# CIawevy/FreeFine

Measured on AMD Instinct MI355X. Metric: edited images/sec/GPU @512px 50-step DDIM, higher is better.
Workload: dtype bf16x3

## Files before the change

### __graft_entry__.py

```python
import os
import subprocess
import sys

ROOT = os.path.dirname(os.path.abspath(__file__))
if ROOT not in sys.path:
    sys.path.insert(0, ROOT)

HIPCC = os.environ.get("HIPCC", "/opt/rocm/bin/hipcc")
LIB = os.path.join(ROOT, "freefine_amd", "libfreefine_hip.so")
CSRC = os.path.join(ROOT, "freefine_amd", "csrc")
OBJDIR = os.path.join(ROOT, "build", "obj")
UNITS = [("capi_igemm.hip", []), ("capi_attn.hip", []), ("capi.hip", []), ("capi_splat.hip", []),
         ("attn_x3w.hip", ["-mllvm", "-amdgpu-mfma-vgpr-form", "-fno-slp-vectorize"]), ("attn_causal.hip", []), ("dift.hip", []), ("imgprep.hip", []),
         ("inception.hip", [])]
COMMON = ["--offload-arch=gfx950", "-O3", "-std=c++17", "-fPIC"]


def _stale(target, deps):
    if not os.path.exists(target):
        return True
    t = os.path.getmtime(target)
    return any(os.path.getmtime(d) > t for d in deps)


def build(force=False):
    deps = [os.path.join(CSRC, f) for f in os.listdir(CSRC)] + [os.path.join(ROOT, "include", "freefine_hip.h")]
    if force or _stale(LIB, deps):
        os.makedirs(OBJDIR, exist_ok=True)
        procs = []
        for src, extra in UNITS:
            obj = os.path.join(OBJDIR, src.replace(".hip", ".o"))
            cmd = [HIPCC] + COMMON + extra + ["-c", "-o", obj, os.path.join(CSRC, src)]
            print("[build]", " ".join(cmd), flush=True)
            procs.append((cmd, obj, subprocess.Popen(cmd, cwd=ROOT)))
        for cmd, obj, pr in procs:
            if pr.wait() != 0:
                raise subprocess.CalledProcessError(pr.returncode, cmd)
        cmd = [HIPCC, "--offload-arch=gfx950", "-shared", "-fPIC", "-o", LIB] + [obj for _, obj, _ in procs]
        print("[build]", " ".join(cmd), flush=True)
        subprocess.check_call(cmd, cwd=ROOT)
    import freefine_amd
    from freefine_amd import _lib
    _lib.load()
    import oracle.attention_modulation, oracle.masks, oracle.pipeline, oracle.scheduler, oracle.sd_unet, oracle.sd_vae
    print(f"[build] {LIB} exports {len(_lib.SYMBOLS)} symbols; oracle importable", flush=True)


def smoke():
    import numpy as np
    import torch
    assert torch.cuda.is_available(), "smoke() needs a GPU"
    from freefine_amd import _lib
    _lib.load()
    sys.path.insert(0, os.path.join(ROOT, "tests"))
    from golden_cases import edit_cases, mask_inputs, oracle_pipe, synth_images
    from test_pipeline_gpu import make_pipe
    dev = torch.device("cuda:0")
    ori_img, coarse, _ = synth_images()
    ori, tgt, *_ = mask_inputs()
    name, unet_name, kw = edit_cases()[0]
    kw = dict(kw)
    text, gs, eta = kw.pop("guidance_text"), kw.pop("guidance_scale"), kw.pop("eta")
    model = make_pipe(dev, unet_name, "edit", graph=True)
    img = model.FreeFine_generation(ori_img, ori, coarse, tgt, text, gs, eta, verbose=True, seed=42, return_intermediates=True, **kw)
    with torch.no_grad():
        o_img, _, o_traj = oracle_pipe(unet_name).freefine_generation(ori_img, ori, coarse, tgt, text, gs, eta, seed=42, **kw)
    dev_max = max((a.float().cpu() - b).abs().max().item() for a, b in zip(model.last_intermediates, o_traj))
# ... 10 lines not shown
```

### freefine_amd/_lib.py

```python
import ctypes as C
import os

_HERE = os.path.dirname(os.path.abspath(__file__))
LIB_PATH = os.environ.get("FREEFINE_HIP_LIB") or os.path.join(_HERE, "libfreefine_hip.so")

FFN_F32, FFN_BF16, FFN_BF16X3, FFN_FP8 = 0, 1, 2, 3
IG_OUT_SILU, IG_OUT_F32, IG_GEGLU, IG_OUT_TRANSPOSED, IG_OUT_PAIR, IG_OUT_GELU, IG_OUT_RELU, IG_OUT_KV64 = 1, 2, 4, 8, 16, 32, 64, 128
IG_OUT_QGELU = 256
ELT_RELU, ELT_ADD, ELT_GELU = 0, 1, 2
ATT_MAXP, ATT_MAXB = 4, 16
ATT_HEAD_RULE, ATT_UNIFORM_SEL1, ATT_UNIFORM_SEL0, ATT_CAUSAL = 1, 2, 4, 8
NORM_SILU, NORM_OUT_PAIR = 1, 2
IMGPREP_MAX_SIDE = 4096
IMGPREP_MAX_TAPS = 2 * 3 * IMGPREP_MAX_SIDE + 1
BOX_NMS_MAX = 16384
KEEP_NONE, KEEP_SUM_LT128, KEEP_GT128 = 0, 1, 2
CHAIN_MAXL, CHAIN_MAXW = 8, 1024
CONV_RELU = 1
POOL_MAX, POOL_AVG_VALID = 0, 1


class IgemmDesc(C.Structure):
    _fields_ = [
        ("A", C.c_void_p), ("W", C.c_void_p), ("out", C.c_void_p),
# ... 67 lines not shown
    ]


class CoarseEditDesc(C.Structure):
    _fields_ = [
        ("src_img", C.c_void_p), ("src_mask", C.c_void_p), ("bg", C.c_void_p), ("hole_img", C.c_void_p), ("hole_mask", C.c_void_p), ("inv", C.c_void_p),
        ("final_img", C.c_void_p), ("tmask", C.c_void_p), ("trans_hole", C.c_void_p),
        ("B", C.c_int), ("H", C.c_int), ("W", C.c_int), ("mask_c", C.c_int), ("hole_mask_c", C.c_int),
    ]


class Conv2dDesc(C.Structure):
    _fields_ = [
        ("x", C.c_void_p), ("w", C.c_void_p), ("bias", C.c_void_p), ("out", C.c_void_p),
        ("B", C.c_int), ("Hin", C.c_int), ("Win", C.c_int), ("Cin", C.c_int), ("N", C.c_int),
        ("KH", C.c_int), ("KW", C.c_int), ("stride", C.c_int), ("pad_h", C.c_int), ("pad_w", C.c_int),
        ("ldx", C.c_int), ("ldo", C.c_int), ("Kpad", C.c_int), ("flags", C.c_int),
    ]


_vp, _i, _f, _l = C.c_void_p, C.c_int, C.c_float, C.c_long
SYMBOLS = {
    "ffn_version": (_i, []),
    "ffn_last_error": (C.c_char_p, []),
    "ffn_device_info": (_i, [_i, C.c_char_p, _i]),
    "ffn_graph_launch": (_i, [_vp, _vp]),
    "ffn_igemm": (_i, [_vp, _i, C.POINTER(IgemmDesc)]),
    "ffn_conv3x3_n4": (_i, [_vp, _i, _vp, _vp, _vp, _vp, _i, _i, _i, _i]),
    "ffn_split_pair": (_i, [_vp, _vp, _vp, _l, _i, _i]),
    "ffn_groupnorm_f8": (_i, [_vp, _vp, _vp, _vp, _vp, _i, _i, _i, _i, _i, _f, _i, _f, _vp, _vp, _vp]),
    "ffn_attn": (_i, [_vp, _i, C.POINTER(AttnDesc)]),
    "ffn_attn_kernel_name": (_i, [_i, C.POINTER(AttnDesc), C.c_char_p, _i]),
    "ffn_igemm_tune": (_i, [_vp, _i, C.POINTER(IgemmDesc)]),
    "ffn_igemm_tune_entry_ints": (_i, []),
    "ffn_igemm_tune_export": (_i, [C.POINTER(C.c_int), _i]),
    "ffn_igemm_tune_import": (_i, [C.POINTER(C.c_int), _i]),
    "ffn_igemm_tune_stamp": (_i, []),
    "ffn_igemm_tune_clear": (_i, []),
    "ffn_igemm_tune_enable": (_i, [_i]),
    "ffn_igemm_num_configs": (_i, []),
    "ffn_igemm_force_config": (_i, [_i]),
    "ffn_igemm_kernel_name": (_i, [_i, C.POINTER(IgemmDesc), C.c_char_p, _i]),
    "ffn_attn_presplit": (_i, [_vp, _vp, _vp, _vp, _vp, _i, _i, _i, _i, _i]),
    "ffn_attn_variant": (_i, [_i, _i, C.POINTER(C.c_int), C.POINTER(C.c_int)]),
    "ffn_gn_nchunk": (_i, [_i]),
    "ffn_gn_fused": (_i, [_i, _i, _i, _i]),
    "ffn_gn_stats": (_i, [_vp, _i, _vp, _vp, _vp, _i, _i, _i, _i, _f, _vp, _vp, _vp]),
    "ffn_gn_apply": (_i, [_vp, _i, _vp, _vp, _vp, _vp, _i, _i, _i, _i]),
    "ffn_groupnorm": (_i, [_vp, _i, _vp, _vp, _vp, _vp, _i, _i, _i, _i, _f, _i, _vp, _vp, _vp]),
    "ffn_groupnorm_pair_raw": (_i, [_vp, _vp, _vp, _vp, _vp, _vp, _i, _i, _i, _i, _f, _i, _vp, _vp, _vp]),
    "ffn_layernorm": (_i, [_vp, _i, _vp, _vp, _vp, _vp, _i, _i, _f]),
    "ffn_layernorm_pair": (_i, [_vp, _vp, _vp, _vp, _vp, _i, _i, _f]),
    "ffn_softmax_rows": (_i, [_vp, _i, _vp, _vp, _l, _i, _f]),
    "ffn_pool_layernorm": (_i, [_vp, _i, _vp, _vp, _vp, _vp, _vp, _i, _i, _i, _f, _i]),
    "ffn_cosine_rows": (_i, [_vp, _vp, _vp, _vp, _i, _i, _i]),
    "ffn_cfg_masked": (_i, [_vp, _vp, _vp, _vp, _f, _vp, _l, _i]),
    "ffn_ddim_inv_step": (_i, [_vp, _vp, _vp, _f, _f, _f, _f, _vp, _vp, _l]),
    "ffn_ddim_ctrl_step": (_i, [_vp, C.POINTER(CtrlStepDesc)]),
    "ffn_pack_nchw": (_i, [_vp, _i, C.POINTER(PackDesc)]),
    "ffn_nhwc_to_nchw_f32": (_i, [_vp, _vp, _vp, _i, _i, _i, _i]),
    "ffn_concat": (_i, [_vp, _i, _vp, _vp, _vp, _l, _i, _i]),
    "ffn_timestep_embed": (_i, [_vp, _i, _vp, _vp, _vp, _i, _i, _i]),
    "ffn_transpose": (_i, [_vp, _i, _vp, _vp, _i, _i, _i, _i, _i]),
    "ffn_cast": (_i, [_vp, _i, _i, _vp, _vp, _l]),
    "ffn_eltwise": (_i, [_vp, _i, _i, _vp, _vp, _vp, _l]),
    "ffn_resize_bilinear": (_i, [_vp, _i, _vp, _vp, _i, _i, _i, _i, _i, _i, _i]),
    "ffn_splat_lift": (_i, [_vp, _vp, _vp, _vp, _i, _i, _i, _f, _f]),
    "ffn_splat_project": (_i, [_vp, _vp, _vp, _i, C.POINTER(SplatXform)]),
    "ffn_splat_bin": (_i, [_vp, _i, _vp, _i, _f, _i, _i, _vp, _vp, _vp]),
    "ffn_splat_render": (_i, [_vp, _vp, _vp, _vp, _vp, _f, _i, _i, _i, _vp, _vp, _vp]),
    "ffn_splat_ids": (_i, [_vp, _vp, _vp, _vp, _f, _i, _i, _i, _vp]),
    "ffn_splat_correspond": (_i, [_vp, _vp, _vp, _i, _i, _i, _vp, _i, _vp, _vp]),
    "ffn_geo_project": (_i, [_vp, _vp, C.POINTER(C.c_float), _f, _i, _i, _vp, _vp]),
    "ffn_splat_composite": (_i, [_vp, _vp, _vp, _vp, _vp, _f, _f, _i, _i, _i, _i, _i, _vp]),
    "ffn_mesh_cover": (_i, [_vp, _vp, _vp, _i, _i, _vp]),
    "ffn_embed_tokens": (_i, [_vp, _i, _vp, _vp, _vp, _vp, _l, _i, _i, _i]),
    "ffn_embed_tokens_ln": (_i, [_vp, _i, _vp, _vp, _vp, _vp, _vp, _vp, _l, _i, _i, _i, _f]),
    "ffn_affine_chain": (_i, [_vp, _vp, _vp, _vp, _i, _i, C.POINTER(C.c_int), _i, _f, _f]),
    "ffn_dift_match": (_i, [_vp, C.POINTER(DiftDesc)]),
    "ffn_dift_workspace_bytes": (_l, [_i, _i, _i, _i]),
    "ffn_sift_base": (_i, [_vp, _vp, _vp, _i, _i, _i]),
    "ffn_gauss_blur_f32": (_i, [_vp, _vp, _vp, _vp, _i, _i, _vp, _i]),
    "ffn_decimate2_f32": (_i, [_vp, _vp, _vp, _i, _i]),
    "ffn_sift_extrema": (_i, [_vp, _vp, _vp, _i, _i, _vp, _i, _vp, C.POINTER(C.c_int)]),
    "ffn_sift_refine_orient": (_i, [_vp, _vp, _vp, _i, _i, _i, _vp, _i, _vp]),
    "ffn_sift_describe": (_i, [_vp, _vp, _i, _i, _i, _vp, _i, _vp, _vp]),
    "ffn_knn2_u8": (_i, [_vp, _vp, _i, _vp, _i, _vp, _vp]),
    "ffn_resize_pil_bilinear_u8": (_i, [_vp, _vp, _vp, _vp, _i, _i, _i, _i, _i, _vp, _vp, _i, _vp, _vp, _i]),
    "ffn_resize_pil_u8": (_i, [_vp, C.POINTER(ResizePilDesc)]),
    "ffn_resize_taps8_u8": (_i, [_vp, _vp, _vp, _i, _i, _i, _i, _i, _i, _vp, _vp, _vp, _vp]),
    "ffn_resize_gather_u8": (_i, [_vp, _vp, _vp, _i, _i, _i, _i, _i, _i, _vp, _vp, _i]),
    "ffn_dilate_u8": (_i, [_vp, _vp, _vp, _vp, _i, _i, _i, _i, _i]),
    "ffn_mask_bbox_u8": (_i, [_vp, _vp, _vp, _i, _i, _i, _i]),
    "ffn_coarse_edit_2d": (_i, [_vp, C.POINTER(CoarseEditDesc)]),
    "ffn_vit_patch_rows": (_i, [_vp, _i, _vp, _vp, _vp, _i, _i, _i, _i, _i]),
    "ffn_vit_patch_rows_pair": (_i, [_vp, _vp, _vp, _vp, _i, _i, _i, _i, _i]),
    "ffn_sam_patch_rows": (_i, [_vp, _i, _vp, _vp, _i, _i, _i, _i, _i, _i, C.POINTER(C.c_float), C.POINTER(C.c_float)]),
    "ffn_sam_patch_rows_pair": (_i, [_vp, _vp, _vp, _i, _i, _i, _i, _i, _i, C.POINTER(C.c_float), C.POINTER(C.c_float)]),
    "ffn_hyper_masks": (_i, [_vp, _vp, _vp, _vp, _i, _i, _i, _i]),
    "ffn_upsample_bicubic": (_i, [_vp, _vp, _vp, _vp, _i, _i, _i, _i, _i]),
    "ffn_upsample_bicubic_stats": (_i, [_vp, _vp, _vp, _vp, _i, _i, _i, _i, _i, _f]),
    "ffn_box_nms": (_i, [_vp, _vp, _vp, _i, _f]),
    "ffn_image_to_nhwc": (_i, [_vp, _i, _vp, _vp, _l, _i]),
    "ffn_nhwc_to_image": (_i, [_vp, _i, _vp, _vp, _i, _i, _i]),
    "ffn_conv2d": (_i, [_vp, _i, C.POINTER(Conv2dDesc)]),
    "ffn_pool2d": (_i, [_vp, _i, _vp, _vp, _i, _i, _i, _i, _i, _i, _i, _i, _i]),
# ... 33 lines not shown
```

### freefine_amd/csrc/capi.hip

```cpp
#include <stdlib.h>
#include <string.h>

#include "capi_common.h"
#include "conv_small.h"
#include "elementwise.h"
#include "norms.h"

__thread char g_err[512] = "";

extern "C" int ffn_version(void) { return 16; }
extern "C" const char* ffn_last_error(void) { return g_err; }
extern "C" int ffn_device_info(int device, char* name, int name_len) {
    hipDeviceProp_t prop;
    hipError_t e = hipGetDeviceProperties(&prop, device);
    if (e != hipSuccess) return fail(FFN_EHIP, "hipGetDeviceProperties: %s", hipGetErrorString(e));
    if (name && name_len > 0) {
        strncpy(name, prop.gcnArchName, name_len - 1);
        name[name_len - 1] = 0;
    }
    return prop.multiProcessorCount;
}

extern "C" int ffn_graph_launch(void* stream, void* graph_exec) {
    REQUIRE(graph_exec, "graph_launch: null graph");
    hipError_t e = hipGraphLaunch(reinterpret_cast<hipGraphExec_t>(graph_exec), reinterpret_cast<hipStream_t>(stream));
    if (e != hipSuccess) return fail(FFN_EHIP, "hipGraphLaunch: %s", hipGetErrorString(e));
    return FFN_OK;
}

extern "C" int ffn_split_pair(void* stream, const float* src, void* dst, long rows, int C, int ld_src) {
    REQUIRE(src && dst && rows > 0 && C > 0 && C % 4 == 0 && ld_src >= C && ld_src % 4 == 0, "split_pair: bad arguments (C=%d, ld_src=%d)", C, ld_src);
    REQUIRE(aligned16(src) && aligned16(dst), "split_pair: pointers must be 16-byte aligned");
    if (C % 8 == 0) LAUNCH(split_pair8_kernel, dim3(grid_for(rows * (C / 8))), dim3(256), 0, reinterpret_cast<hipStream_t>(stream), src, (bf16*)dst, rows, C, ld_src);
    else LAUNCH(split_pair_kernel, dim3(grid_for(rows * (C / 4))), dim3(256), 0, reinterpret_cast<hipStream_t>(stream), src, (bf16*)dst, rows, C, ld_src);
    return check_launch("split_pair");
}
extern "C" int ffn_conv3x3_n4(void* stream, int dtype, const void* x, const float* w, const float* bias, float* out, int B, int H, int W, int Cin) {
    REQUIRE(dtype == FFN_F32 || dtype == FFN_BF16, "conv3x3_n4: fp32 or bf16 activations");
    REQUIRE(x && w && out && aligned16(x) && aligned16(w) && aligned16(out) && (!bias || aligned16(bias)), "conv3x3_n4: null / unaligned pointer");
    REQUIRE(B > 0 && H > 0 && W > 0 && Cin > 0 && Cin % 16 == 0 && Cin <= 448, "conv3x3_n4: B=%d H=%d W=%d Cin=%d (Cin %% 16 == 0, <= 448)", B, H, W, Cin);
    hipStream_t s = reinterpret_cast<hipStream_t>(stream);
    const long npix = (long)B * H * W;
    const int lds = 36 * Cin * 4;
    dim3 grid((unsigned)((npix + 63) / 64));
    int rc;
    if (dtype == FFN_F32) {
        if ((rc = set_lds(conv3x3_n4_kernel<float>, lds))) return rc;
        LAUNCH(conv3x3_n4_kernel<float>, grid, dim3(256), lds, s, (const float*)x, w, bias, out, B, H, W, Cin);
    } else {
        if ((rc = set_lds(conv3x3_n4_kernel<bf16>, lds))) return rc;
        LAUNCH(conv3x3_n4_kernel<bf16>, grid, dim3(256), lds, s, (const bf16*)x, w, bias, out, B, H, W, Cin);
    }
    return check_launch("conv3x3_n4");
}

extern "C" int ffn_eltwise(void* stream, int dtype, int op, const void* a, const void* b, void* y, long n) {
    REQUIRE(dtype == FFN_F32 || dtype == FFN_BF16, "eltwise: bad dtype %d", dtype);
    REQUIRE(op == FFN_ELT_RELU || op == FFN_ELT_ADD || op == FFN_ELT_GELU, "eltwise: bad op %d", op);
    REQUIRE(a && y && (op != FFN_ELT_ADD || b), "eltwise: null operand");
    REQUIRE(n > 0 && n % 4 == 0, "eltwise: n=%ld must be a positive multiple of 4", n);
    hipStream_t s = reinterpret_cast<hipStream_t>(stream);
    const long n4 = n / 4;
    const int grid = grid_for(n4);
// ... 274 lines not shown
```

### freefine_amd/ops.py

```python
import ctypes as CT
import math

import os
import threading

import torch

from . import _lib as L


def _dt(t):
    if t.dtype == torch.float32:
        return L.FFN_F32
    if t.dtype == torch.bfloat16:
        return L.FFN_BF16
    raise TypeError(f"unsupported dtype {t.dtype}")


def epc(dtype):
    return 4 if dtype == torch.float32 else 8


def kstage(dtype):
    return 8 * epc(dtype)
# ... 302 lines not shown
    d.a_lo = (32 if d.x3 == 2 else K) if x3 else 0
    odt = torch.float32 if x3 else x.dtype
    d.rows_per_batch = rows_per_batch or M
    d.ldrb = rowbias.stride(0) if rowbias is not None else 0
    flags = 0
    n_out = N
    if silu:
        flags |= L.IG_OUT_SILU
    if gelu:
        flags |= L.IG_OUT_GELU
    if relu:
        flags |= L.IG_OUT_RELU
    if qgelu:
        flags |= L.IG_OUT_QGELU
    if geglu:
        flags |= L.IG_GEGLU
        n_out = N // 2
    if out_f32:
        flags |= L.IG_OUT_F32
    if transposed_ld is not None:
        flags |= L.IG_OUT_TRANSPOSED
        nb = M // d.rows_per_batch
        if out is None:
            alloc = torch.zeros if transposed_ld > d.rows_per_batch else torch.empty
            out = alloc(nb, N, transposed_ld, dtype=odt, device=x.device)
        d.ldo = transposed_ld
    elif out_pair:
        assert x3 and out is None
        flags |= L.IG_OUT_PAIR
        out = _mark_pair(torch.empty(*x.shape[:-1], 2 * n_out, dtype=torch.bfloat16, device=x.device), n_out)
        d.ldo = 2 * n_out
    else:
        if out is None:
            out = torch.empty(*x.shape[:-1], n_out, dtype=torch.float32 if out_f32 else odt, device=x.device)
        d.ldo = out.stride(-2) if out.ndim > 1 else n_out
    assert xa.stride(-1) == 1 and out.stride(-1) == 1 and (residual is None or residual.stride(-1) == 1), "linear: x, out and residual need contiguous columns"
    d.ldr = (residual.stride(-2) if residual.ndim > 1 else residual.shape[-1]) if residual is not None else 0
    d.out = out.data_ptr()
    if kv64_from is not None:
        assert x3 and residual is None and rowbias is None and not (silu or gelu or relu or qgelu or geglu or out_pair)
        flags |= L.IG_OUT_KV64
        d.kv64_from = int(kv64_from)
        splitk = 1
    d.flags, d.alpha, d.conv = flags, alpha, 0
    if splitk == 0 and _invariant():
        splitk = 1
    d.splitk, d.ws, d.ws_bytes = splitk, _workspace(x.device).data_ptr(), WS_BYTES
    if _PROF is None:
        L.check(lib.ffn_igemm(_stream(), dcode, CT.byref(d)), "ffn_igemm")
    else:
        esz = x.element_size()
        L.check(_timed(_igemm_name(lib, dcode, d), 2.0 * M * N * K, esz * (M * K + N * K + M * n_out),
                       lambda: lib.ffn_igemm(_stream(), dcode, CT.byref(d))), "ffn_igemm")
    return out


def conv3x3(x, w, bias, B, Hin, Win, Cin, *, stride=1, pad=1, upsample=False, out=None, residual=None, rowbias=None,
            rowbias_ld=None, out_f32=False, Hout=None, Wout=None, splitk=0, relu=False):
    lib = L.load()
    He, We = (Hin * 2, Win * 2) if upsample else (Hin, Win)
    if Hout is None:
        Hout = (He + 2 * pad - 3) // stride + 1
        Wout = (We + 2 * pad - 3) // stride + 1
    N = w.shape[0]
    d = L.IgemmDesc()
    x3 = is_x3(w)
    f8 = is_f8(w)
    if f8:
        assert x.dtype == torch.uint8 and x.shape[-1] == w._ffn_f8[0] and out_f32 is False
        Cin = x.shape[-1]
        xa = x
    elif x3 and pair_width(x) is not None:
        assert pair_width(x) == Cin
        xa = x
    else:
        xa = split_pair(x, Cin) if x3 else x
    dcode = L.FFN_FP8 if f8 else (L.FFN_BF16X3 if x3 else _dt(x))
    odt = torch.float32 if x3 else (torch.bfloat16 if f8 else x.dtype)
    d.A, d.W = xa.data_ptr(), w.data_ptr()
    d.bias, d.rowbias, d.residual = _p(bias), _p(rowbias), _p(residual)
    d.M, d.N, d.K, d.Kpad = B * Hout * Wout, N, 9 * Cin, w.shape[1]
    d.lda = 2 * Cin if x3 else Cin
    d.x3 = int(w._ffn_x3) if x3 else 0
    d.a_lo = (32 if d.x3 == 2 else Cin) if x3 else 0
    d.rows_per_batch = Hout * Wout
    d.ldrb = (rowbias_ld or rowbias.stride(0)) if rowbias is not None else 0
    if out is None:
        out = torch.empty(B, Hout * Wout, N, dtype=torch.float32 if out_f32 else odt, device=x.device)
    assert xa.is_contiguous(), "conv3x3: x must be contiguous (a column view of a wider buffer has no pixel stride the kernels could follow)"
    assert out.stride(-1) == 1 and (residual is None or residual.stride(-1) == 1), "conv3x3: out and residual need contiguous columns"
    d.out, d.ldo = out.data_ptr(), out.stride(-2)
    d.ldr = residual.stride(-2) if residual is not None else 0
    d.Hin, d.Win, d.Cin, d.Hout, d.Wout = Hin, Win, Cin, Hout, Wout
    d.stride, d.pad, d.upsample = stride, pad, 1 if upsample else 0
    d.flags, d.alpha, d.conv = (L.IG_OUT_F32 if out_f32 else 0) | (L.IG_OUT_RELU if relu else 0), (w._ffn_f8[1] if f8 else 1.0), 1
    if splitk == 0 and _invariant():
        splitk = 1
    d.splitk, d.ws, d.ws_bytes = splitk, _workspace(x.device).data_ptr(), WS_BYTES
    if _PROF is None:
        L.check(lib.ffn_igemm(_stream(), dcode, CT.byref(d)), "ffn_igemm(conv)")
    else:
        esz = x.element_size()
        k_real = 9 * getattr(x, "_ffn_f8_act", Cin)
        L.check(_timed(_igemm_name(lib, dcode, d), 2.0 * d.M * N * k_real, esz * (x.numel() + N * d.K + d.M * N),
                       lambda: lib.ffn_igemm(_stream(), dcode, CT.byref(d))), "ffn_igemm(conv)")
    return out
# ... 1143 lines not shown
```

### freefine_amd/unet.py

```python
import ctypes as CT
import weakref

import torch

from . import _lib as L
from . import ops
from .config import UNetConfig


class _Res:
    pass


class HipUNet:
    def __init__(self, cfg: UNetConfig, state, dtype=torch.bfloat16, device="cuda:0", x3=False, fp8_conv=False):
        assert not x3 or dtype == torch.float32, "split-bf16 mode keeps fp32 activations"
        assert not fp8_conv or dtype == torch.bfloat16, "fp8 convolutions are an option of the bf16 fast mode"
        self.x3 = bool(x3)
        self.fp8_conv = bool(fp8_conv)
        self.cfg, self.dtype, self.device = cfg, dtype, torch.device(device)
        self.in_channels = cfg.in_channels
        self.hook, self.controller = "edit", None
        self._graphs = {}
        self._capture_stream = None
# ... 534 lines not shown
            vt2 = torch.cat([vt[..., :Sk], vt[rr][..., :Sk]], dim=2).contiguous()
            return ops.attention(q, k2, vt2, t.heads, scale, plan["passes"], Sk=2 * Sk, C=t.C, x3=self.x3, out_pair=self.x3)
        return ops.attention(q, k, vt, t.heads, scale, plan["passes"], Sk=Sk, C=t.C, w_dev=self.cg_dev if plan["needs_cg"] else None, x3=self.x3,
                             out_pair=self.x3, kv_images=kv_images)

    def _kv_buffers(self, B, S, C, ldv):
        ru = self._reuse
        i = ru["cursor"]
        ru["cursor"] = i + 1
        if ru.get("static_ready"):
            return ru["static_bufs"][i]
        k_ref, vt_ref = ru["state"][2 * i], ru["state"][2 * i + 1]
        nr = k_ref.shape[0]
        assert tuple(k_ref.shape) == (nr, S, C) and tuple(vt_ref.shape) == (nr, C, ldv), (tuple(k_ref.shape), tuple(vt_ref.shape), (S, C, ldv))
        qk = torch.empty(B + nr, S, 2 * C, dtype=self.dtype, device=self.device)
        vt = torch.empty(B + nr, C, ldv, dtype=self.dtype, device=self.device)
        qk[B:, :, C:].copy_(k_ref)
        vt[B:].copy_(vt_ref)
        if ru.get("static") is not None:
            ru["static_bufs"].append((qk, vt))
            ru["static"] += [qk[B:, :, C:], vt[B:]]
        return qk, vt

    def _transformer_block(self, t, x, B, H, W, place, kv_text, out=None, drop=None, tb=0):
        S, C = H * W, t.C
        res0 = x
        ru = self._reuse
        h = self._gn(x, t.norm, 1e-6, False)
        h = ops.linear(h, t.proj_in[0], t.proj_in[1], K=C)
        y = ops.layernorm(h, *t.ln[0], pair=self.x3)
        ldv = (S + 7) // 8 * 8
        if ru is not None and ru["mode"] == "replay_kv" and tb >= ru["kv_from"]:
            qk, vt = self._kv_buffers(B, S, C, ldv)
            ops.linear(y, t.w_qk1, None, K=C, out=qk[:B])
            ops.linear(y, t.w_v1, None, K=C, rows_per_batch=S, transposed_ld=ldv, out=vt[:B])
            self._kv_ext = True
            a = self._attention(t, False, place, qk[:B], qk[..., C:], vt, 2 * C, B, S, S, plan=self._self_plan(t, place, B, S))
            self._kv_ext = False
        else:
            plan = self._self_plan(t, place, B, S, drop_ref_queries=drop is not None)
            rec = ru is not None and ru["mode"] == "record" and ru.get("kv_from") is not None and tb >= ru["kv_from"]
            img = self.x3 and not rec and (plan is None or plan["kind"] != "shared_kv") and \
                ops.kv_images_ok(C // t.heads, S, S, None if plan is None else plan["passes"], B * max(S * 2 * C, C * ldv) * 4)
            qk = ops.linear(y, t.w_qk1, None, K=C, kv64_from=C if img else None)
            vt = ops.linear(y, t.w_v1, None, K=C, rows_per_batch=S, transposed_ld=ldv, kv64_from=0 if img else None)
            if rec:
                self.last_kv.append((qk[..., C:], vt))
            a = self._attention(t, False, place, qk, qk[..., C:], vt, 2 * C, B, S, S, plan=plan, kv_images=img)
        if drop is not None:
            idx, kv_text = drop
            h, res0, B = h.index_select(0, idx), res0.index_select(0, idx), idx.shape[0]
            self._in_phase_a = True
        h = ops.linear(a, t.o1[0], t.o1[1], K=C, residual=h)
        y = ops.layernorm(h, *t.ln[1], pair=self.x3)
        q = ops.linear(y, t.w_q2, None, K=C)
        k2, vt2 = kv_text
        a = self._attention(t, True, place, q, k2, vt2, C, B, S, k2.shape[1])
        h = ops.linear(a, t.o2[0], t.o2[1], K=C, residual=h)
        y = ops.layernorm(h, *t.ln[2], pair=self.x3)
        y = ops.linear(y, t.ff1[0], t.ff1[1], K=C, geglu=True, out_pair=self.x3)
        h = ops.linear(y, t.ff2[0], t.ff2[1], K=4 * C, residual=h, out_pair=self.x3 and C % 32 == 0)
        return ops.linear(h, t.proj_out[0], t.proj_out[1], K=C, residual=res0, out=out)

    def _run(self, sample, text_kv, stop_up=None):
        cfg = self.cfg
        B, _, H, W = sample.shape
        dt = self.dtype
        ru = self._reuse
        replay = ru is not None and ru["mode"] == "replay"
        record = ru is not None and ru["mode"] == "record"
        replay_kv = ru is not None and ru["mode"] == "replay_kv"
        BB = B
        if replay:
            sample = sample.index_select(0, ru["idx_a"])
            B = sample.shape[0]
            text_kv = list(ru["text_kv_a"][:self.join_block_tb(ru["join"])]) + list(text_kv[self.join_block_tb(ru["join"]):])
        if replay_kv:
            sample = sample.index_select(0, ru["idx_a"])
            B = sample.shape[0]
            text_kv = ru["text_kv_a"]
            ru["cursor"] = 0
        if record and ru.get("kv_from") is not None:
            self.last_kv = []
        self._in_phase_a = replay
        ti = iter(text_kv)
        tb = 0
        te = ops.timestep_embed(self.t_dev, self.freq, BB, dt, flip=cfg.flip_sin_to_cos)
        e1 = ops.linear(te, self.te1[0], self.te1[1], K=self.te1[2], silu=True)
        e2 = ops.linear(e1, self.te2[0], self.te2[1], K=self.te2[2], silu=True)
        temb_all = ops.linear(e2, self.temb_w, self.temb_b, K=self.te2[0].shape[0], out_f32=True)
        temb_full = temb_all
        temb_all = temb_all[:B]
        x = ops.pack_nchw(sample, list(range(B)), self.cin_pad, dt)
        x = ops.conv3x3(x, self.conv_in[0], self.conv_in[1], B, H, W, self.cin_pad)
        skips = [(x, H, W)]
        n = len(self.down)
        for i, blk in enumerate(self.down):
            for j, r in enumerate(blk.res):
                x = self._resblock(r, x, B, H, W, temb_all)
                if blk.attn:
                    x = self._transformer_block(blk.attn[j], x, B, H, W, "down", next(ti), tb=tb)
                    tb += 1
                skips.append((x, H, W))
            if blk.down is not None:
                C = x.shape[-1]
                x = ops.conv3x3(x, blk.down[0], blk.down[1], B, H, W, C, stride=2)
                H, W = (H + 1) // 2, (W + 1) // 2
                skips.append((x, H, W))
# ... 54 lines not shown
```

### include/freefine_hip.h

```cpp
#ifndef FREEFINE_HIP_H
#define FREEFINE_HIP_H
#include <stdint.h>
#ifdef __cplusplus
extern "C" {
#endif

enum { FFN_F32 = 0, FFN_BF16 = 1, FFN_BF16X3 = 2 ,
       FFN_FP8 = 3  };
enum { FFN_OK = 0, FFN_EINVAL = -22, FFN_ENOSYS = -38, FFN_EHIP = -5, FFN_ENOSPC = -28 };

int ffn_version(void);
const char* ffn_last_error(void);
int ffn_device_info(int device, char* name, int name_len);
int ffn_graph_launch(void* stream, void* graph_exec);

enum {
    FFN_IG_OUT_SILU = 1 << 0,
    FFN_IG_OUT_F32 = 1 << 1,
    FFN_IG_GEGLU = 1 << 2,
    FFN_IG_OUT_TRANSPOSED = 1 << 3,
    FFN_IG_OUT_PAIR = 1 << 4,
    FFN_IG_OUT_GELU = 1 << 5,
    FFN_IG_OUT_KV64 = 1 << 7,
    FFN_IG_OUT_RELU = 1 << 6,
// ... 55 lines not shown
    const void* k;
    const void* vt;
    void* out;
    const float* w_dev;
    int Bo, S, Sk, heads, D;
    int ldq, ldk, ldvt, ldo;
    float scale;
    int npass;
    int out_pair;
    int kv_pair;
    ffn_attn_entry e[FFN_ATT_MAXP * FFN_ATT_MAXB];
} ffn_attn_desc;
int ffn_attn(void* stream, int dtype, const ffn_attn_desc* d);
int ffn_attn_presplit(void* stream, const float* k, const float* vt, void* k_pair, void* vt_pair, int rows, int Sk, int heads, int ldk, int ldvt);
int ffn_attn_variant(int dtype, int D, int* dp, int* qf);
int ffn_attn_kernel_name(int dtype, const ffn_attn_desc* d, char* buf, int len);

enum { FFN_ELT_RELU = 0, FFN_ELT_ADD = 1, FFN_ELT_GELU = 2 };
int ffn_eltwise(void* stream, int dtype, int op, const void* a, const void* b, void* y, long n);
int ffn_resize_bilinear(void* stream, int dtype, const void* x, void* y, int B, int Hin, int Win, int Hout, int Wout, int C, int relu);

typedef struct ffn_splat_xform {
    float center[3], translate[3], rotate[9] , scale[3];
    float tan_half_fov;
} ffn_splat_xform;
int ffn_splat_lift(void* stream, const float* depth, const int* idx, float* pts, int n, int W, int H, float fx, float fy);
int ffn_splat_project(void* stream, const float* pts, float* proj, int n, const ffn_splat_xform* x);
int ffn_splat_bin(void* stream, int fill, const float* proj, int n, float radius, int W, int H, int* counts, const int* offs, int* list);
int ffn_splat_render(void* stream, const float* proj, const float* rgb, const int* offs, const int* list, float radius, int K, int W, int H,
                     float* image, int* idx_sum, uint8_t* covered);
int ffn_splat_ids(void* stream, const float* proj, const int* offs, const int* list, float radius, int K, int W, int H, int* ids);
int ffn_splat_correspond(void* stream, const float* proj, const int* idx, int n, int W, int H, const int* ids, int K, float* map, uint8_t* visible);

int ffn_geo_project(void* stream, const float* depth, const float* pose, float focal, int H, int W, float* tcoords, float* proj);
int ffn_splat_composite(void* stream, const float* proj, const float* feat, const int* offs, const int* list, float radius, float tau, int K,
                        int C, int H, int W, int round_half, float* out);
int ffn_mesh_cover(void* stream, const float* tcoords, const uint8_t* mask, int H, int W, uint8_t* cover);

enum { FFN_NORM_SILU = 1, FFN_NORM_OUT_PAIR = 2 };
int ffn_gn_nchunk(int HW);
int ffn_gn_fused(int B, int HW, int C, int G);
int ffn_gn_stats(void* stream, int dtype, const void* x, const float* gamma, const float* beta, int B, int HW, int C, int G,
                 float eps, float* partial_ws, float* scale, float* shift);
int ffn_gn_apply(void* stream, int dtype, const void* x, void* y, const float* scale, const float* shift, int B, int HW,
                 int C, int silu);
int ffn_groupnorm(void* stream, int dtype, const void* x, void* y, const float* gamma, const float* beta, int B, int HW, int C, int G,
                  float eps, int silu, float* partial_ws, float* scale, float* shift);
int ffn_groupnorm_pair_raw(void* stream, const void* x, void* y_pair, void* yraw_pair, const float* gamma, const float* beta, int B, int HW, int C, int G,
                           float eps, int silu, float* partial_ws, float* scale, float* shift);
int ffn_layernorm(void* stream, int dtype, const void* x, void* y, const float* gamma, const float* beta, int M, int C,
                  float eps);
int ffn_layernorm_pair(void* stream, const float* x, void* y, const float* gamma, const float* beta, int M, int C, float eps);
int ffn_softmax_rows(void* stream, int dtype, const void* x, void* y, long M, int N, float scale);
int ffn_pool_layernorm(void* stream, int dtype, const void* x, const int* ids, void* y, const float* gamma, const float* beta, int N, int S, int C, float eps,
                       int pair);
int ffn_cosine_rows(void* stream, const float* a, const float* b, float* out, int B, int P, int b_rows);

int ffn_cfg_masked(void* stream, const float* eps_u, const float* eps_c, const float* mask, float cfg, float* eps, long n,
                   int HW);
int ffn_ddim_inv_step(void* stream, const float* eps, const float* x, float c_bt, float c_at, float c_an, float c_bn,
                      float* x_next, float* pred_x0, long n);
typedef struct ffn_ctrl_step_desc {
    const float* eps;
    const float* x;
    const float* noise;
    const float* m;
    const float* om;
    float* x_prev;
    float* pred_x0;
    float c_bt, c_at, c_ap, c_dir;
    float c_dirm[8], stdv[8];
    int row_masked[8];
    int rows, CHW, HW;
} ffn_ctrl_step_desc;
int ffn_ddim_ctrl_step(void* stream, const ffn_ctrl_step_desc* d);

typedef struct ffn_pack_desc {
    const float* src;
    void* dst;
    int src_row[16];
    int B, Cl, CP, HW;
} ffn_pack_desc;
int ffn_pack_nchw(void* stream, int dtype, const ffn_pack_desc* d);
int ffn_nhwc_to_nchw_f32(void* stream, const float* src, float* dst, int B, int HW, int C, int ld);
int ffn_concat(void* stream, int dtype, const void* a, const void* b, void* out, long rows, int C1, int C2);
int ffn_timestep_embed(void* stream, int dtype, const float* t_dev, const float* freq, void* out, int B, int half, int flip);
int ffn_transpose(void* stream, int dtype, const void* src, void* dst, int B, int R, int C, int ld_src, int ld_dst);
int ffn_cast(void* stream, int src_dtype, int dst_dtype, const void* src, void* dst, long n);
int ffn_embed_tokens(void* stream, int dtype, const int* ids, const float* table, const float* pos, void* out, long M, int S, int C, int V);
int ffn_embed_tokens_ln(void* stream, int dtype, const int* ids, const float* table, const float* pos, void* out, const float* gamma, const float* beta, long M,
                        int S, int C, int V, float eps);
#define FFN_CHAIN_MAXL 8
#define FFN_CHAIN_MAXW 1024
int ffn_affine_chain(void* stream, const float* x, const float* params, float* out, int B, int ldx, const int* dims, int L, float shift, float scale);
int ffn_image_to_nhwc(void* stream, int dtype, const uint8_t* img, void* dst, long npix, int CP);
int ffn_nhwc_to_image(void* stream, int dtype, const void* src, float* dst, int B, int HW, int ld);

typedef struct ffn_dift_desc {
    const void* src;
    const void* tgt;
    const int* kps;
    void* ws;
    int* out_rc;
    float* out_cos;
    long ws_bytes;
    long es;
// ... 88 lines not shown
```

Before: 1.976.

## Fuse LayerNorm into the cross-attention Q projection GEMM for C=320

Adds a dedicated kernel that computes LayerNorm on fp32 rows, splits the result into bf16 hi/lo pairs held in registers (AGPR/VGPR), and runs a bf16x3 MFMA GEMM against the Q weight. The weight is streamed through a three-slot LDS ring using buffer-to-LDS loads. The UNet transformer block uses it for the cross-attention query when the hidden width is 320. This removes the separate layernorm kernel and the round trip of the normalized pair tensor through memory. In exchange it adds a hand-scheduled kernel with a K restricted to 320, tight register pressure and explicit waitcnt tuning.

```diff
diff --git a/__graft_entry__.py b/__graft_entry__.py
--- a/__graft_entry__.py
+++ b/__graft_entry__.py
@@ -12,7 +12,7 @@
 OBJDIR = os.path.join(ROOT, "build", "obj")
 UNITS = [("capi_igemm.hip", []), ("capi_attn.hip", []), ("capi.hip", []), ("capi_splat.hip", []),
          ("attn_x3w.hip", ["-mllvm", "-amdgpu-mfma-vgpr-form", "-fno-slp-vectorize"]), ("attn_causal.hip", []), ("dift.hip", []), ("imgprep.hip", []),
-         ("inception.hip", [])]
+         ("inception.hip", []), ("igemm_as.hip", ["-mllvm", "-amdgpu-mfma-vgpr-form", "-fno-slp-vectorize"])]
 COMMON = ["--offload-arch=gfx950", "-O3", "-std=c++17", "-fPIC"]
 
 
diff --git a/freefine_amd/_lib.py b/freefine_amd/_lib.py
--- a/freefine_amd/_lib.py
+++ b/freefine_amd/_lib.py
@@ -143,6 +143,7 @@
     "ffn_layernorm": (_i, [_vp, _i, _vp, _vp, _vp, _vp, _i, _i, _f]),
     "ffn_layernorm_pair": (_i, [_vp, _vp, _vp, _vp, _vp, _i, _i, _f]),
     "ffn_softmax_rows": (_i, [_vp, _i, _vp, _vp, _l, _i, _f]),
+    "ffn_ln_igemm": (_i, [_vp, _vp, _i, _vp, _vp, _f, _i, _i, _vp, _i, _vp, _i, _vp, _i]),
     "ffn_pool_layernorm": (_i, [_vp, _i, _vp, _vp, _vp, _vp, _vp, _i, _i, _i, _f, _i]),
     "ffn_cosine_rows": (_i, [_vp, _vp, _vp, _vp, _i, _i, _i]),
     "ffn_cfg_masked": (_i, [_vp, _vp, _vp, _vp, _f, _vp, _l, _i]),
diff --git a/freefine_amd/csrc/capi.hip b/freefine_amd/csrc/capi.hip
--- a/freefine_amd/csrc/capi.hip
+++ b/freefine_amd/csrc/capi.hip
@@ -8,7 +8,7 @@
 
 __thread char g_err[512] = "";
 
-extern "C" int ffn_version(void) { return 16; }
+extern "C" int ffn_version(void) { return 17; }
 extern "C" const char* ffn_last_error(void) { return g_err; }
 extern "C" int ffn_device_info(int device, char* name, int name_len) {
     hipDeviceProp_t prop;
diff --git a/freefine_amd/csrc/igemm_as.h b/freefine_amd/csrc/igemm_as.h
--- /dev/null
+++ b/freefine_amd/csrc/igemm_as.h
@@ -0,0 +1,237 @@
+#pragma once
+#include "common.h"
+
+typedef __attribute__((ext_vector_type(16))) float f32x16;
+typedef __attribute__((address_space(3))) void* as_lptr_t;
+
+struct LnIgemmParams {
+    const float* x;
+    const float* gamma;
+    const float* beta;
+    const void* W;
+    const float* bias;
+    void* out;
+    int M, N, ldx, Kpad, ldo;
+    int wbytes, obytes;
+    float eps;
+};
+
+#define LNIG_SB_FREE (0x002 | 0x004 | 0x010 | 0x020 | 0x040 | 0x400)
+constexpr int LNIG_SLOT = 10 * 4096;
+constexpr int LNIG_RING = 3;
+constexpr int LNIG_OFF_B = LNIG_RING * LNIG_SLOT;
+constexpr int LNIG_STG_ROW = 1296, LNIG_STG_WAVE = 16 * LNIG_STG_ROW;
+constexpr int LNIG_LDS = LNIG_OFF_B + 4 * LNIG_RING * 256;
+static_assert(4 * LNIG_STG_WAVE <= LNIG_LDS, "the prologue's staging area lies over the ring");
+
+__device__ __forceinline__ void lnig_row_load(const float* x, long row, long ldx, int C, int lane, u32x4 (&v)[2]) {
+    const int cch = C / 4;
+#pragma unroll
+    for (int i = 0; i < 2; ++i) {
+        const int cc = lane + 64 * i;
+        v[i] = *reinterpret_cast<const u32x4*>(x + row * ldx + (cc < cch ? cc : 0) * 4);
+    }
+}
+template <int NR>
+__device__ __forceinline__ void lnig_rows_to_lds(const u32x4 (&v)[NR][2], const float (&gam)[2][4], const float (&bet)[2][4], int C, float eps, int lane, char* dst) {
+    constexpr int EPC = 4;
+    const bool two = lane + 64 < C / EPC;
+    float f[NR][2][EPC], s[NR], ss[NR];
+#pragma unroll
+    for (int r = 0; r < NR; ++r) {
+        s[r] = 0.f;
+#pragma unroll
+        for (int i = 0; i < 2; ++i) {
+            DT<float>::unpack(v[r][i], f[r][i]);
+#pragma unroll
+            for (int e = 0; e < EPC; ++e) s[r] = (i == 0 || two) ? s[r] + f[r][i][e] : s[r];
+        }
+    }
+    for (int off = 32; off > 0; off >>= 1)
+#pragma unroll
+        for (int r = 0; r < NR; ++r) s[r] += __shfl_xor(s[r], off);
+#pragma unroll
+    for (int r = 0; r < NR; ++r) {
+        const float mean = s[r] / (float)C;
+        s[r] = mean;
+        ss[r] = 0.f;
+#pragma unroll
+        for (int i = 0; i < 2; ++i)
+#pragma unroll
+            for (int e = 0; e < EPC; ++e) {
+#pragma clang fp contract(off)
+                const float d = f[r][i][e] - mean;
+                const float t = ss[r] + d * d;
+                ss[r] = (i == 0 || two) ? t : ss[r];
+            }
+    }
+    for (int off = 32; off > 0; off >>= 1)
+#pragma unroll
+        for (int r = 0; r < NR; ++r) ss[r] += __shfl_xor(ss[r], off);
+#pragma unroll
+    for (int r = 0; r < NR; ++r) {
+        const float mean = s[r];
+        const float rstd = 1.0f / sqrtf(ss[r] / (float)C + eps);
+#pragma unroll
+        for (int i = 0; i < 2; ++i) {
+            float o[EPC];
+#pragma unroll
+            for (int e = 0; e < EPC; ++e) o[e] = (f[r][i][e] - mean) * rstd * gam[i][e] + bet[i][e];
+            u32x2 hi, lo;
+            hi[0] = pack_bf16x2(o[0], o[1]);
+            hi[1] = pack_bf16x2(o[2], o[3]);
+            lo[0] = pack_bf16x2(o[0] - __uint_as_float(hi[0] << 16), o[1] - __uint_as_float(hi[0] & 0xffff0000u));
+            lo[1] = pack_bf16x2(o[2] - __uint_as_float(hi[1] << 16), o[3] - __uint_as_float(hi[1] & 0xffff0000u));
+            char* row = dst + r * LNIG_STG_ROW;
+            const int cc = lane + 64 * i;
+            *reinterpret_cast<u32x2*>(row + ((i == 0 || two) ? cc * 8 : 1280)) = hi;
+            *reinterpret_cast<u32x2*>(row + ((i == 0 || two) ? 640 + cc * 8 : 1288)) = lo;
+        }
+    }
+}
+
+__global__ __launch_bounds__(256) void ln_igemm_as_kernel(const LnIgemmParams p) {
+    constexpr int C = 320, KS = C / 16, NKB = C / 32;
+    constexpr int OOB = (int)0x80000000;
+    extern __shared__ __attribute__((aligned(16))) char smem[];
+    const int tid = threadIdx.x, lane = tid & 63, wave = __builtin_amdgcn_readfirstlane(tid >> 6);
+    const int r = lane & 31, h = lane >> 5;
+    const int mt = blockIdx.x * 256;
+    const int mw = mt + wave * 64;
+
+    u32x4 xh[2][KS], xl[2][KS];
+    {
+        char* stg = smem + wave * LNIG_STG_WAVE;
+        float gam[2][4], bet[2][4];
+#pragma unroll
+        for (int i = 0; i < 2; ++i) {
+            const int cc = lane + 64 * i < C / 4 ? lane + 64 * i : 0;
+            load4(p.gamma + 4 * cc, gam[i]);
+            load4(p.beta + 4 * cc, bet[i]);
+        }
+#pragma unroll
+        for (int sl = 0; sl < 4; ++sl) {
+#pragma unroll
+            for (int half = 0; half < 2; ++half) {
+                u32x4 xv[8][2];
+#pragma unroll
+                for (int rr = 0; rr < 8; ++rr) {
+                    int row = mw + sl * 16 + half * 8 + rr;
+                    row = row < p.M ? row : p.M - 1;
+                    lnig_row_load(p.x, (long)row, (long)p.ldx, C, lane, xv[rr]);
+                }
+                lnig_rows_to_lds<8>(xv, gam, bet, C, p.eps, lane, stg + half * 8 * LNIG_STG_ROW);
+            }
+            __builtin_amdgcn_wave_barrier();
+            if ((r >> 4) == (sl & 1)) {
+                const char* src = stg + (r & 15) * LNIG_STG_ROW + 16 * h;
+#pragma unroll
+                for (int s = 0; s < KS; ++s) {
+                    xh[sl >> 1][s] = *reinterpret_cast<const u32x4*>(src + 32 * s);
+                    xl[sl >> 1][s] = *reinterpret_cast<const u32x4*>(src + 640 + 32 * s);
+                }
+            }
+            __builtin_amdgcn_wave_barrier();
+            if (sl & 1) {
+#pragma unroll
+                for (int s = 0; s < KS; ++s) {
+                    asm volatile("" : "+a"(xh[sl >> 1][s]));
+                    if (sl == 1) asm volatile("" : "+a"(xl[0][s]));
+                    else asm volatile("" : "+v"(xl[1][s]));
+                }
+            }
+        }
+    }
+
+    const int nch = p.N / 32;
+    const __amdgpu_buffer_rsrc_t rsW = __builtin_amdgcn_make_buffer_rsrc(const_cast<void*>(p.W), 0, p.wbytes, 0x00020000);
+    const __amdgpu_buffer_rsrc_t rsB = __builtin_amdgcn_make_buffer_rsrc(const_cast<float*>(p.bias), 0, p.bias ? p.N * 4 : 0, 0x00020000);
+    const __amdgpu_buffer_rsrc_t rsO = __builtin_amdgcn_make_buffer_rsrc(p.out, 0, p.obytes, 0x00020000);
+    const int lr = lane >> 3;
+    const int w_voff = (8 * wave + lr) * p.Kpad * 2 + (((lane & 7) ^ (4 * (wave & 1) + (lr >> 1))) << 4);
+    const int b_voff = lane < 32 ? lane * 4 : OOB;
+    auto dma_chunk = [&](int c, int slot) {
+        const bool valid = c < nch;
+        char* dst = smem + slot * LNIG_SLOT + wave * 1024;
+        const int so = valid ? c * 32 * p.Kpad * 2 : 0;
+        const int vo_ = valid ? w_voff : OOB;
+#pragma unroll
+        for (int kb = 0; kb < NKB; ++kb) __builtin_amdgcn_raw_ptr_buffer_load_lds(rsW, (as_lptr_t)(dst + kb * 4096), 16, vo_, so + kb * 128, 0, 0);
+        __builtin_amdgcn_raw_ptr_buffer_load_lds(rsB, (as_lptr_t)(smem + LNIG_OFF_B + (wave * LNIG_RING + slot) * 256), 4, valid ? b_voff : OOB, valid ? c * 128 : 0, 0, 0);
+    };
+    int rdh[2], rdl[2];
+#pragma unroll
+    for (int s2 = 0; s2 < 2; ++s2) {
+        rdh[s2] = r * 128 + (((2 * s2 + h) ^ ((r >> 1) & 7)) << 4);
+        rdl[s2] = r * 128 + (((4 + 2 * s2 + h) ^ ((r >> 1) & 7)) << 4);
+    }
+    int vo[2];
+#pragma unroll
+    for (int rb = 0; rb < 2; ++rb) {
+        const int lrow = wave * 64 + rb * 32 + r;
+        vo[rb] = mt + lrow < p.M ? (lrow * p.ldo + 4 * h) * 4 : OOB;
+    }
+
+    f32x16 acc[2];
+    auto store_chunk = [&](int c, bool live) {
+#pragma unroll
+        for (int rb = 0; rb < 2; ++rb) {
+            const int vo_ = live ? vo[rb] : OOB;
+#pragma unroll
+            for (int q = 0; q < 4; ++q) {
+                const u32x4 w = {__float_as_uint(acc[rb][4 * q]), __float_as_uint(acc[rb][4 * q + 1]), __float_as_uint(acc[rb][4 * q + 2]), __float_as_uint(acc[rb][4 * q + 3])};
+                __builtin_amdgcn_raw_buffer_store_b128(w, rsO, vo_, (mt * p.ldo + 32 * c + 8 * q) * 4, 0);
+            }
+        }
+    };
+
+    __syncthreads();
+    dma_chunk(0, 0);
+    dma_chunk(1, 1);
+    asm volatile("s_waitcnt vmcnt(11)" ::: "memory");
+    __builtin_amdgcn_s_barrier();
+    asm volatile("" ::: "memory");
+    int slot = 0;
+    for (int c = 0; c < nch; ++c) {
+        const int nslot = slot == 0 ? 2 : slot - 1;
+        dma_chunk(c + 2, nslot);
+        store_chunk(c - 1, c > 0);
+        const char* img0 = smem + slot * LNIG_SLOT;
+        {
+            const char* bs = smem + LNIG_OFF_B + (wave * LNIG_RING + slot) * 256 + 16 * h;
+#pragma unroll
+            for (int q = 0; q < 4; ++q) {
+                const f32x4 b = *reinterpret_cast<const f32x4*>(bs + 32 * q);
+#pragma unroll
+                for (int rb = 0; rb < 2; ++rb) {
+                    acc[rb][4 * q] = b[0]; acc[rb][4 * q + 1] = b[1]; acc[rb][4 * q + 2] = b[2]; acc[rb][4 * q + 3] = b[3];
+                }
+            }
+        }
+        u32x4 fw[4][2];
+        auto rd_w = [&](int s_, int buf) {
+            const char* img = img0 + (s_ >> 1) * 4096;
+            fw[buf][0] = *reinterpret_cast<const u32x4*>(img + rdh[s_ & 1]);
+            fw[buf][1] = *reinterpret_cast<const u32x4*>(img + rdl[s_ & 1]);
+        };
+        rd_w(0, 0); rd_w(1, 1); rd_w(2, 2);
+#pragma unroll
+        for (int s = 0; s < KS; ++s) {
+            if (s + 3 < KS) rd_w(s + 3, (s + 3) & 3);
+            __builtin_amdgcn_sched_barrier(LNIG_SB_FREE);
+            const bf16x8_t wh = __builtin_bit_cast(bf16x8_t, fw[s & 3][0]), wl = __builtin_bit_cast(bf16x8_t, fw[s & 3][1]);
+#pragma unroll
+            for (int rb = 0; rb < 2; ++rb) {
+                acc[rb] = __builtin_amdgcn_mfma_f32_32x32x16_bf16(wl, __builtin_bit_cast(bf16x8_t, xh[rb][s]), acc[rb], 0, 0, 0);
+                acc[rb] = __builtin_amdgcn_mfma_f32_32x32x16_bf16(wh, __builtin_bit_cast(bf16x8_t, xl[rb][s]), acc[rb], 0, 0, 0);
+                acc[rb] = __builtin_amdgcn_mfma_f32_32x32x16_bf16(wh, __builtin_bit_cast(bf16x8_t, xh[rb][s]), acc[rb], 0, 0, 0);
+            }
+            __builtin_amdgcn_sched_barrier(LNIG_SB_FREE);
+        }
+        slot = slot == 2 ? 0 : slot + 1;
+        asm volatile("s_waitcnt vmcnt(19) lgkmcnt(0)" ::: "memory");
+        __builtin_amdgcn_s_barrier();
+        asm volatile("" ::: "memory");
+    }
+    store_chunk(nch - 1, true);
+}
diff --git a/freefine_amd/csrc/igemm_as.hip b/freefine_amd/csrc/igemm_as.hip
--- /dev/null
+++ b/freefine_amd/csrc/igemm_as.hip
@@ -0,0 +1,23 @@
+#include "capi_common.h"
+#include "igemm_as.h"
+
+extern "C" int ffn_ln_igemm(void* stream, const float* x, int ldx, const float* gamma, const float* beta, float eps, int M, int K, const void* W, int Kpad,
+                            const float* bias, int N, float* out, int ldo) {
+    REQUIRE(x && gamma && beta && W && out && M > 0 && N > 0, "ln_igemm: bad arguments");
+    REQUIRE(K == 320, "ln_igemm: K = 320 only (K=%d): the row block's whole contraction stays in registers", K);
+    REQUIRE(N % 32 == 0, "ln_igemm: N must be a multiple of the 32-column chunk (N=%d)", N);
+    REQUIRE(ldx >= K && ldx % 4 == 0 && Kpad >= 2 * K && Kpad % 8 == 0 && aligned16(x) && aligned16(W) && aligned16(out), "ln_igemm: operands need 16-byte aligned rows");
+    REQUIRE(ldo >= N && ldo % 4 == 0, "ln_igemm: ldo=%d too small for N=%d", ldo, N);
+    const long lim = 1L << 31;
+    const long xbytes = ((long)(M - 1) * ldx + K) * 4, wbytes = (long)N * Kpad * 2, obytes = ((long)(M - 1) * ldo + N) * 4;
+    REQUIRE(xbytes < lim && wbytes < lim && obytes < lim && (long)((M + 255) / 256 * 256) * ldo * 4 < lim, "ln_igemm: every operand must stay below 2 GiB");
+    LnIgemmParams p;
+    p.x = x; p.gamma = gamma; p.beta = beta; p.W = W; p.bias = bias; p.out = out;
+    p.M = M; p.N = N; p.ldx = ldx; p.Kpad = Kpad; p.ldo = ldo;
+    p.wbytes = (int)wbytes; p.obytes = (int)obytes; p.eps = eps;
+    hipStream_t s = reinterpret_cast<hipStream_t>(stream);
+    int rc = set_lds(ln_igemm_as_kernel, LNIG_LDS);
+    if (rc != FFN_OK) return rc;
+    LAUNCH(ln_igemm_as_kernel, dim3((M + 255) / 256), dim3(256), LNIG_LDS, s, p);
+    return check_launch("ln_igemm");
+}
diff --git a/freefine_amd/ops.py b/freefine_amd/ops.py
--- a/freefine_amd/ops.py
+++ b/freefine_amd/ops.py
@@ -378,6 +378,27 @@
         esz = x.element_size()
         L.check(_timed(_igemm_name(lib, dcode, d), 2.0 * M * N * K, esz * (M * K + N * K + M * n_out),
                        lambda: lib.ffn_igemm(_stream(), dcode, CT.byref(d))), "ffn_igemm")
+    return out
+
+
+_LN_GEMM = True
+
+
+def ln_gemm_ok(x, w):
+    return _LN_GEMM and is_x3(w) and int(w._ffn_x3) == 2 and x.dtype == torch.float32 and x.shape[-1] == 320 and w.shape[0] % 32 == 0
+
+
+def ln_linear(x, gamma, beta, w, bias=None, *, eps=1e-5):
+    lib = L.load()
+    assert ln_gemm_ok(x, w) and x.stride(-1) == 1 and w.stride(-1) == 1
+    K = x.shape[-1]
+    M = x.numel() // K
+    N = w.shape[0]
+    ldx = x.stride(-2) if x.ndim > 1 else K
+    out = torch.empty(*x.shape[:-1], N, dtype=torch.float32, device=x.device)
+    call = lambda: lib.ffn_ln_igemm(_stream(), x.data_ptr(), ldx, gamma.data_ptr(), beta.data_ptr(), eps, M, K, w.data_ptr(), w.stride(0), _p(bias), N,
+                                    out.data_ptr(), N)
+    L.check(_timed("ln_igemm_as_kernel(LnIgemmParams)", 2.0 * M * N * K, 4.0 * M * K + 4.0 * N * K + 4.0 * M * N, call), "ffn_ln_igemm")
     return out
 
 
diff --git a/freefine_amd/unet.py b/freefine_amd/unet.py
--- a/freefine_amd/unet.py
+++ b/freefine_amd/unet.py
@@ -610,8 +610,11 @@
             h, res0, B = h.index_select(0, idx), res0.index_select(0, idx), idx.shape[0]
             self._in_phase_a = True
         h = ops.linear(a, t.o1[0], t.o1[1], K=C, residual=h)
-        y = ops.layernorm(h, *t.ln[1], pair=self.x3)
-        q = ops.linear(y, t.w_q2, None, K=C)
+        if ops.ln_gemm_ok(h, t.w_q2):
+            q = ops.ln_linear(h, *t.ln[1], t.w_q2)
+        else:
+            y = ops.layernorm(h, *t.ln[1], pair=self.x3)
+            q = ops.linear(y, t.w_q2, None, K=C)
         k2, vt2 = kv_text
         a = self._attention(t, True, place, q, k2, vt2, C, B, S, k2.shape[1])
         h = ops.linear(a, t.o2[0], t.o2[1], K=C, residual=h)
diff --git a/include/freefine_hip.h b/include/freefine_hip.h
--- a/include/freefine_hip.h
+++ b/include/freefine_hip.h
@@ -131,6 +131,8 @@
                   float eps);
 int ffn_layernorm_pair(void* stream, const float* x, void* y, const float* gamma, const float* beta, int M, int C, float eps);
 int ffn_softmax_rows(void* stream, int dtype, const void* x, void* y, long M, int N, float scale);
+int ffn_ln_igemm(void* stream, const float* x, int ldx, const float* gamma, const float* beta, float eps, int M, int K, const void* W, int Kpad,
+                 const float* bias, int N, float* out, int ldo);
 int ffn_pool_layernorm(void* stream, int dtype, const void* x, const int* ids, void* y, const float* gamma, const float* beta, int N, int S, int C, float eps,
                        int pair);
 int ffn_cosine_rows(void* stream, const float* a, const float* b, float* out, int B, int P, int b_rows);
```

Result: no change. 1.980, median of 2 (+0.2%).
